# wamuumu/query-recommendation-system

Measured on AMD Instinct MI355X. Metric: MinHash signatures/sec through the whole hot path (signatures -> LSH candidates -> pair scoring -> top-K), higher is better.
Workload: dtype u16/int32 MinHash values, uint64 keys and pairs (integer); float64 cosine

## Files before the change

query-recommendation-system_amd/csrc/bucket.hip:

```cpp
#include "common.h"


struct PartPool {
  uint64_t *keys;
  uint32_t *vals;
  unsigned long long *cursor;
  uint32_t cap;
  uint4 *runs;
  unsigned long long *nruns;
  uint32_t runs_max;
  uint32_t *fill;
  uint32_t slot_base;
};

#ifndef QR_PS_IPT
#define QR_PS_IPT 16
#endif
constexpr int PS_IPT = QR_PS_IPT;
constexpr int PS_TILE = SORT_THREADS * PS_IPT;
constexpr int PS_WGS = PS_IPT <= 16 ? 3 : 2;
template <bool LEVEL2>
__global__ __launch_bounds__(SORT_THREADS, PS_WGS) void part_scatter_atomic_kernel(
    const uint64_t *__restrict__ keys_in, const uint32_t *__restrict__ vals_in, uint64_t *__restrict__ keys_out,
    uint32_t *__restrict__ vals_out, int64_t n_in, int ntiles, int shift, uint32_t dmask,
    uint32_t *__restrict__ cursors, uint32_t cap, uint32_t *__restrict__ overflow, uint64_t ek,
    const uint32_t *__restrict__ in_counts, uint32_t in_cap, int64_t chunk_len, int64_t chunk_stride,
    int64_t band_stride, PartPool pool) {
  __shared__ uint32_t cnt[RADIX];
  __shared__ uint32_t lsum[SORT_THREADS / WAVE];
  __shared__ uint32_t gdelta[RADIX];
  __shared__ uint8_t gok[RADIX];
  __shared__ uint64_t skey[PS_TILE];
  __shared__ uint32_t sval[PS_TILE];
  const int tile = LEVEL2 ? (int)blockIdx.x : xcd_tile(blockIdx.x, ntiles), batch = blockIdx.y;
  const int lane = threadIdx.x & (WAVE - 1), w = threadIdx.x >> 6;
  const int64_t n = LEVEL2 ? (int64_t)min(in_counts[batch], in_cap) : n_in;
  const int64_t tbase = (int64_t)tile * PS_TILE;
  if (tbase >= n) return;
  cnt[threadIdx.x] = 0;
  __syncthreads();
  const size_t boff = LEVEL2 ? (size_t)batch * in_cap : (size_t)batch * (size_t)(band_stride ? band_stride : n);
  const bool chunked = !LEVEL2 && chunk_len > 0 && chunk_len < n;
  const int64_t wbase = tbase + (int64_t)w * (WAVE * PS_IPT);
  const uint32_t nd = dmask + 1u;
  uint64_t key[PS_IPT];
  uint32_t val[PS_IPT];
  uint32_t dr[PS_IPT];
#pragma unroll
  for (int k = 0; k < PS_IPT; ++k) {
    const int64_t idx = wbase + (int64_t)k * WAVE + lane;
    const size_t at = chunked ? boff + (size_t)(idx / chunk_len) * chunk_stride + (size_t)(idx % chunk_len) : boff + idx;
    key[k] = idx < n ? keys_in[at] : ek;
    val[k] = LEVEL2 ? (idx < n ? vals_in[boff + idx] : 0u) : (uint32_t)idx;
  }
#pragma unroll
  for (int k = 0; k < PS_IPT; ++k) {
    const int64_t idx = wbase + (int64_t)k * WAVE + lane;
    const bool valid = idx < n && (LEVEL2 || key[k] != ek);
    if (!LEVEL2) key[k] = qr_mix64(key[k]);
    const uint32_t d = (uint32_t)(key[k] >> shift) & dmask;
    dr[k] = valid ? (d << 16) | atomicAdd(&cnt[d], 1u) : 0xFFFFFFFFu;
  }
  __syncthreads();
  const uint32_t tc = cnt[threadIdx.x];
  const uint32_t gb = tc ? atomicAdd(&cursors[(size_t)batch * nd + threadIdx.x], tc) : 0u;
  uint32_t lstart;
  {
    const uint32_t linc = wave_incl_scan(tc);
    if (lane == WAVE - 1) lsum[w] = linc;
    __syncthreads();
    lstart = linc - tc;
#pragma unroll
    for (int k = 0; k < SORT_THREADS / WAVE; ++k)
      if (k < w) lstart += lsum[k];
    cnt[threadIdx.x] = lstart;
  }
  __syncthreads();
#pragma unroll
  for (int k = 0; k < PS_IPT; ++k) {
    if (dr[k] != 0xFFFFFFFFu) {
      const uint32_t lp = cnt[dr[k] >> 16] + (dr[k] & 0xFFFFu);
      skey[lp] = key[k];
      sval[lp] = val[k];
    }
  }
  {
    const int d = threadIdx.x;
    uint32_t where = gb + tc <= cap ? 1u : 0u;
    uint32_t delta = (uint32_t)d * cap + gb - lstart;
    if (!where) {
      if (pool.keys) {
        const unsigned long long pb =
            __hip_atomic_fetch_add(pool.cursor, (unsigned long long)tc, __ATOMIC_RELAXED, __HIP_MEMORY_SCOPE_AGENT);
        if (pb + tc <= (unsigned long long)pool.cap) {
          const unsigned long long ri = __hip_atomic_fetch_add(pool.nruns, 1ull, __ATOMIC_RELAXED, __HIP_MEMORY_SCOPE_AGENT);
          if (ri < (unsigned long long)pool.runs_max) {
            const uint32_t slot = pool.slot_base + (uint32_t)batch * nd + (uint32_t)d;
            pool.runs[ri] = make_uint4(slot, tc, (uint32_t)pb, 0u);
            atomicMin(&pool.fill[slot], gb);
            where = 2u;
            delta = (uint32_t)pb - lstart;
          }
        }
      }
      if (!where) atomicOr(overflow, 1u);
    }
    gok[d] = (uint8_t)where;
    gdelta[d] = delta;
  }
  __syncthreads();
  uint32_t nstaged = 0;
#pragma unroll
  for (int k = 0; k < SORT_THREADS / WAVE; ++k) nstaged += lsum[k];
  const size_t obase = (size_t)batch * nd * cap;
#pragma unroll
  for (int k = 0; k < PS_IPT; ++k) {
    const uint32_t p = k * SORT_THREADS + threadIdx.x;
    if (p < nstaged) {
      const uint64_t x = skey[p];
      const uint32_t d = (uint32_t)(x >> shift) & dmask;
      const uint32_t where = gok[d];
      if (where == 1u) {
        const size_t dst = obase + (uint32_t)(gdelta[d] + p);
        keys_out[dst] = x;
        vals_out[dst] = sval[p];
      } else if (where == 2u) {
        const uint32_t dst = gdelta[d] + p;
        pool.keys[dst] = x;
        pool.vals[dst] = sval[p];
      }
    }
  }
}

#ifndef QR_FIN_THREADS
#define QR_FIN_THREADS 1024
#endif
#ifndef QR_FIN_CAP
#define QR_FIN_CAP 6144
#endif
constexpr int FIN_THREADS = QR_FIN_THREADS;
constexpr int FIN_CAP = QR_FIN_CAP;
constexpr int FIN_IPT = FIN_CAP / FIN_THREADS;
constexpr int FIN_SMALL_THREADS = 512, FIN_SMALL_CAP = 4096;
constexpr int FIN_SMALL_MEAN = 2800;

template <int CAP = FIN_CAP> __device__ static inline uint32_t fin_home(uint64_t key) {
  uint32_t h = (uint32_t)key * 0x9E3779B1u;
  h ^= h >> 15;
  h += (uint32_t)(key >> 32) * 0x85EBCA77u;
  h ^= h >> 13;
  h *= 0xC2B2AE3Du;
  return __umulhi(h, (uint32_t)CAP);
}

#ifndef QR_FIN_COOP
#define QR_FIN_COOP 16
#endif
constexpr uint32_t FIN_COOP = QR_FIN_COOP;
__device__ static inline void emit_run(uint64_t *__restrict__ dst, uint32_t pos, uint32_t me, const uint32_t *run,
                                       uint32_t run_off, uint32_t c) {
  if (c <= FIN_COOP) {
    for (uint32_t t = 0; t < c; ++t) {
      const uint32_t other = run[run_off + t];
      dst[pos + t] = (uint64_t)min(me, other) << 32 | max(me, other);
    }
  }
  uint64_t big = __ballot(c > FIN_COOP);
  const int lane = threadIdx.x & (WAVE - 1);
// ... 59 lines not shown

template <int IPT>
__device__ static inline void fin_layout(const uint32_t (&so)[IPT], const uint32_t (&ireg)[IPT], const uint32_t *start,
                                         uint32_t *grp) {
#pragma unroll
  for (int j = 0; j < IPT; ++j)
    if (so[j] != 0xFFFFFFFFu) grp[start[so[j] & 0xFFFFu] + (so[j] >> 16)] = ireg[j];
}

template <int IPT>
__device__ static inline void fin_emit(uint64_t *__restrict__ dst, uint32_t pos, const uint32_t (&so)[IPT],
                                       const uint32_t (&ireg)[IPT], const uint32_t *start, const uint32_t *grp) {
#pragma unroll
  for (int j = 0; j < IPT; ++j) {
    const bool rec = so[j] != 0xFFFFFFFFu;
    const uint32_t o = rec ? so[j] >> 16 : 0u;
    emit_run(dst, pos, ireg[j], grp, rec ? start[so[j] & 0xFFFFu] : 0u, o);
    pos += o;
  }
}

template <int THREADS = FIN_THREADS, int CAP = FIN_CAP>
__global__ __launch_bounds__(THREADS, THREADS >= 1024 ? 8 : 6) void bucket_finish_kernel(
    const uint64_t *__restrict__ keys, const uint32_t *__restrict__ ids, int nparts, uint64_t ek, uint64_t *__restrict__ blk,
    uint32_t *__restrict__ overflow, uint64_t *__restrict__ out, uint64_t capacity, const uint32_t *__restrict__ counts,
    uint32_t cap, uint64_t *__restrict__ biglist, unsigned long long *__restrict__ nbig, uint32_t big_max,
    uint32_t big_base) {
  constexpr int IPT = CAP / THREADS;
  static_assert(CAP % THREADS == 0 && CAP <= 65535, "image = whole records per thread, slots fit 16 bits");
  __shared__ unsigned long long gbase;
  __shared__ __attribute__((aligned(16))) unsigned long long tab[CAP];
  __shared__ uint32_t cnt[CAP];
  __shared__ uint32_t wsum[THREADS / WAVE];
  const int part = blockIdx.x, band = blockIdx.y;
  const int tid = threadIdx.x;
  const size_t bslot = (size_t)band * nparts + part;
  const uint32_t m = counts[bslot];
  const size_t first = bslot * cap;
  if (m > (uint32_t)CAP || m > cap) {
    if (tid == 0) fin_list_part(big_base + bslot, biglist, nbig, big_max, overflow);
    return;
  }
  if (m == 0) return;
  const uint64_t *k = keys + first;
  const uint32_t *id = ids + first;
  uint64_t kreg[IPT];
  uint32_t ireg[IPT];
#pragma unroll
  for (int j = 0; j < IPT; ++j) {
    const uint32_t i = tid + j * THREADS;
    kreg[j] = i < m ? k[i] : ek;
    ireg[j] = i < m ? id[i] : 0u;
  }
#pragma unroll
  for (int j = 0; j < IPT; ++j) {
    const uint32_t i = tid + j * THREADS;
    tab[i] = ek;
    cnt[i] = 0;
  }
  __syncthreads();
  uint32_t so[IPT];
  uint32_t mine = 0;
  uint32_t slot[IPT];
  unsigned long long seen[IPT];
#pragma unroll
  for (int j = 0; j < IPT; ++j) {
    slot[j] = fin_home<CAP>(kreg[j]);
    seen[j] = kreg[j] != ek
                  ? atomicCAS(&tab[slot[j]], (unsigned long long)ek, (unsigned long long)kreg[j])
                  : (unsigned long long)ek;
  }
#pragma unroll
  for (int j = 0; j < IPT; ++j) {
    if (kreg[j] != ek) {
      unsigned long long old = seen[j];
      while (old != ek && old != kreg[j]) {
        slot[j] = slot[j] + 1 == (uint32_t)CAP ? 0u : slot[j] + 1;
        old = atomicCAS(&tab[slot[j]], (unsigned long long)ek, (unsigned long long)kreg[j]);
      }
// ... 3 lines not shown
  for (int j = 0; j < IPT; ++j) {
    so[j] = 0xFFFFFFFFu;
    if (kreg[j] != ek) {
      const uint32_t o = atomicAdd(&cnt[slot[j]], 1u);
      so[j] = o << 16 | slot[j];
      mine += o;
    }
  }
  uint32_t tot;
  const uint32_t pos0 = fin_reserve<THREADS>(mine, wsum, blk, &gbase, tot);
  if (tot == 0) return;
  fin_run_starts<THREADS, IPT>([&](uint32_t sl) { return cnt[sl]; }, cnt, wsum);
  __syncthreads();
  uint32_t *grp = reinterpret_cast<uint32_t *>(tab);
  fin_layout(so, ireg, cnt, grp);
  __syncthreads();
  const uint64_t obase = (uint64_t)gbase;
  if (obase + tot > capacity) return;
  fin_emit(out + obase, pos0, so, ireg, cnt, grp);
}

constexpr int FIN_PK_THREADS = 512, FIN_PK_CAP = 4096, FIN_PK_MAX = 4095;
__global__ __launch_bounds__(FIN_PK_THREADS, 8) void bucket_finish_packed_kernel(
    const uint64_t *__restrict__ keys, const uint32_t *__restrict__ ids, int nparts, uint64_t *__restrict__ blk,
    uint32_t *__restrict__ overflow, uint64_t *__restrict__ out, uint64_t capacity, const uint32_t *__restrict__ counts,
    uint32_t cap, uint64_t *__restrict__ biglist, unsigned long long *__restrict__ nbig, uint32_t big_max,
    uint32_t big_base) {
  constexpr int THREADS = FIN_PK_THREADS, CAP = FIN_PK_CAP, IPT = CAP / THREADS;
  constexpr unsigned long long KMASK = (1ull << 52) - 1ull, ONE = 1ull << 52;
  __shared__ unsigned long long gbase;
  __shared__ __attribute__((aligned(16))) unsigned long long tab[CAP];
  __shared__ uint32_t wsum[THREADS / WAVE];
  const int part = blockIdx.x, band = blockIdx.y;
  const int tid = threadIdx.x;
  const size_t bslot = (size_t)band * nparts + part;
  const uint32_t m = counts[bslot];
  if (m > (uint32_t)FIN_PK_MAX) {
    if (tid == 0) fin_list_part(big_base + bslot, biglist, nbig, big_max, overflow);
    return;
  }
  if (m == 0) return;
  const size_t first = bslot * cap;
  const uint64_t *k = keys + first;
  const uint32_t *id = ids + first;
  uint64_t kreg[IPT];
  uint32_t ireg[IPT];
#pragma unroll
  for (int j = 0; j < IPT; ++j) {
    const uint32_t i = tid + j * THREADS;
    kreg[j] = i < m ? k[i] : 0ull;
    ireg[j] = i < m ? id[i] : 0u;
  }
#pragma unroll
  for (int j = 0; j < IPT; ++j) tab[tid + j * THREADS] = 0ull;
  __syncthreads();
  uint32_t so[IPT];
  uint32_t mine = 0;
#pragma unroll
  for (int j = 0; j < IPT; ++j) {
    so[j] = 0xFFFFFFFFu;
    if (tid + j * THREADS < (int)m) {
      const unsigned long long k52 = kreg[j] & KMASK;
      uint32_t slot = fin_home<CAP>(kreg[j]);
      uint32_t o;
      for (;;) {
        const unsigned long long old = atomicCAS(&tab[slot], 0ull, k52 | ONE);
        if (old == 0ull) {
          o = 0;
          break;
        }
        if ((old & KMASK) == k52) {
          o = (uint32_t)(atomicAdd(&tab[slot], ONE) >> 52);
          break;
        }
        slot = slot + 1 == (uint32_t)CAP ? 0u : slot + 1;
      }
      so[j] = o << 16 | slot;
      mine += o;
    }
  }
  uint32_t tot;
  const uint32_t pos0 = fin_reserve<THREADS>(mine, wsum, blk, &gbase, tot);
  if (tot == 0) return;
  uint32_t *rs = reinterpret_cast<uint32_t *>(tab);
  uint32_t *grp = rs + CAP;
  fin_run_starts<THREADS, IPT>([&](uint32_t sl) { return (uint32_t)(tab[sl] >> 52); }, rs, wsum);
  __syncthreads();
  fin_layout(so, ireg, rs, grp);
  __syncthreads();
  const uint64_t obase = (uint64_t)gbase;
  if (obase + tot > capacity) return;
  fin_emit(out + obase, pos0, so, ireg, rs, grp);
}

constexpr int FIN_BIG_GRID = 256;
constexpr int FIN_BIG_BLOCKS = 16;
constexpr uint32_t FIN_BIG_LIST = 4096;
constexpr int FIN_BIG_SLICES = 8;
constexpr int FIN_RANK_SORT = 256;
constexpr uint32_t POOL_RUNS = 1u << 20;

struct BigDesc {
  uint64_t where;
  uint32_t m, pool;
};

__global__ __launch_bounds__(256) void bucket_big_gather_kernel(const uint64_t *__restrict__ biglist,
                                                                const unsigned long long *__restrict__ nbig, uint32_t big_max,
                                                                BigDesc *__restrict__ desc, const uint64_t *__restrict__ part_keys,
                                                                const uint32_t *__restrict__ part_ids,
                                                                const uint32_t *__restrict__ counts, uint32_t cap, PartPool pool,
                                                                uint32_t max_records, uint32_t *__restrict__ overflow) {
  __shared__ unsigned long long base_s;
  __shared__ uint32_t match[256];
  __shared__ uint32_t nmatch;
  const int tid = threadIdx.x;
  unsigned long long nb = *nbig;
  if (nb > big_max) nb = big_max;
  for (unsigned long long e = blockIdx.x; e < nb; e += gridDim.x) {
    const uint32_t slot = (uint32_t)biglist[e];
    const uint32_t m = counts[slot];
    const uint32_t f = pool.fill ? pool.fill[slot] : 0xFFFFFFFFu;
    if (m > max_records || (f == 0xFFFFFFFFu && m > cap)) {
      if (tid == 0) {
        atomicOr(overflow, 1u);
        desc[e] = BigDesc{0ull, 0u, 0u};
      }
      continue;
    }
    if (f == 0xFFFFFFFFu) {
      if (tid == 0) desc[e] = BigDesc{(uint64_t)slot * cap, m, 0u};
      continue;
    }
// ... 22 lines not shown
      __syncthreads();
      const unsigned long long r = r0 + tid;
      if (r < nr && pool.runs[r].x == slot) match[atomicAdd(&nmatch, 1u)] = (uint32_t)r;
      __syncthreads();
      const uint32_t nm = nmatch;
      for (uint32_t q = 0; q < nm; ++q) {
        const uint4 run = pool.runs[match[q]];
        if (at + run.y <= m)
          for (uint32_t i = tid; i < run.y; i += blockDim.x) {
            pool.keys[base + at + i] = pool.keys[(size_t)run.z + i];
            pool.vals[base + at + i] = pool.vals[(size_t)run.z + i];
          }
        at += run.y;
      }
    }
    if (tid == 0) {
      if (at != m) atomicOr(overflow, 1u);
      desc[e] = BigDesc{(uint64_t)base, at == m ? m : 0u, 1u};
    }
  }
}

__global__ __launch_bounds__(FIN_THREADS) void bucket_finish_big_kernel(
    const uint64_t *__restrict__ keys, const uint32_t *__restrict__ ids, const uint64_t *pool_keys, const uint32_t *pool_ids,
    uint64_t ek, const BigDesc *__restrict__ desc, const unsigned long long *__restrict__ nbig, uint32_t big_max,
    uint64_t *__restrict__ blk, uint64_t *__restrict__ out, uint64_t capacity) {
  __shared__ unsigned long long gbase;
  __shared__ __attribute__((aligned(16))) unsigned long long tab[FIN_CAP];
  __shared__ uint32_t cnt[FIN_CAP + 1];
  __shared__ uint32_t grp[FIN_CAP];
  __shared__ uint32_t srt[FIN_CAP];
  __shared__ uint32_t wsum[FIN_THREADS / WAVE];
  __shared__ uint32_t lrun[FIN_CAP / (FIN_RANK_SORT + 1) + 1], nlrun;
  const int tid = threadIdx.x;
  unsigned long long nb = *nbig;
  if (nb > big_max) nb = big_max;
  constexpr int COMBOS = FIN_BIG_BLOCKS * (FIN_BIG_BLOCKS + 1) / 2;
  static_assert(FIN_THREADS % FIN_BIG_SLICES == 0, "a thread's records share their position mod the slice count");
  for (unsigned long long item = blockIdx.x; item < nb * COMBOS * FIN_BIG_SLICES; item += gridDim.x) {
    const uint32_t sl = (uint32_t)(item % FIN_BIG_SLICES);
    const unsigned long long e = item / ((unsigned long long)COMBOS * FIN_BIG_SLICES);
    int combo = (int)((item / FIN_BIG_SLICES) % COMBOS);
    uint32_t bi = 0;
    while (combo > (int)bi) {
      combo -= (int)bi + 1;
      ++bi;
    }
    const uint32_t bj_only = (uint32_t)combo;
    const BigDesc de = desc[e];
    const uint32_t m = de.m;
    const uint64_t *k = (de.pool ? pool_keys : keys) + de.where;
    const uint32_t *id = (de.pool ? pool_ids : ids) + de.where;
    const uint32_t nblk = (m + FIN_CAP - 1) / FIN_CAP;
    if (bi >= nblk) continue;
    {
      const uint32_t lo = bi * FIN_CAP, mb = min((uint32_t)FIN_CAP, m - lo);
      uint64_t kreg[FIN_IPT];
      uint32_t ireg[FIN_IPT], so[FIN_IPT];
      __syncthreads();
#pragma unroll
      for (int j = 0; j < FIN_IPT; ++j) {
        const uint32_t i = tid + j * FIN_THREADS;
        kreg[j] = i < mb ? k[lo + i] : ek;
        ireg[j] = i < mb ? id[lo + i] : 0u;
        tab[i] = ek;
        cnt[i] = 0;
      }
      __syncthreads();
#pragma unroll
      for (int j = 0; j < FIN_IPT; ++j) {
        so[j] = 0xFFFFFFFFu;
        if (kreg[j] != ek) {
          uint32_t slot = fin_home(kreg[j]);
          for (;;) {
            const unsigned long long old = atomicCAS(&tab[slot], (unsigned long long)ek, (unsigned long long)kreg[j]);
            if (old == ek || old == kreg[j]) break;
            slot = slot + 1 == (uint32_t)FIN_CAP ? 0u : slot + 1;
          }
          const uint32_t o = atomicAdd(&cnt[slot], 1u);
          so[j] = o << 16 | slot;
        }
      }
      __syncthreads();
      {
        const uint32_t all = fin_run_starts<FIN_THREADS, FIN_IPT>([&](uint32_t s) { return cnt[s]; }, cnt, wsum);
        if (tid == 0) cnt[FIN_CAP] = all;
      }
// ... 66 lines not shown
        const uint32_t pos0 = block_excl_scan<FIN_THREADS>(mine, wsum, tot);
        if (tid == 0 && tot)
          gbase = __hip_atomic_fetch_add(reinterpret_cast<unsigned long long *>(blk), (unsigned long long)tot,
                                         __ATOMIC_RELAXED, __HIP_MEMORY_SCOPE_AGENT);
        __syncthreads();
        if (tot && gbase + tot <= capacity) {
          uint64_t *dst = out + gbase;
          uint32_t pos = pos0;
#pragma unroll
          for (int j = 0; j < FIN_IPT; ++j) {
            emit_run(dst, pos, ireg[j], srt, so[j] != 0xFFFFFFFFu ? cnt[so[j] & 0xFFFFu] : 0u, rk[j]);
            pos += rk[j];
          }
        }
      }
      if (bj_only < bi) {
        const uint32_t bj = bj_only;
        const uint32_t lo2 = bj * FIN_CAP;
        uint32_t hit[FIN_IPT];
        uint32_t mine2 = 0;
#pragma unroll
        for (int j = 0; j < FIN_IPT; ++j) {
          const uint32_t i = tid + j * FIN_THREADS;
          const uint64_t x = k[lo2 + i];
          ireg[j] = id[lo2 + i];
          uint32_t slot = fin_home(x), found = 0xFFFFFFFFu;
          const bool my_slice = (uint32_t)(tid & (FIN_BIG_SLICES - 1)) == sl;
          for (int step = 0; my_slice && step < FIN_CAP; ++step) {
            const unsigned long long tv = tab[slot];
            if (tv == x) {
              found = slot;
              break;
            }
            if (tv == ek) break;
            slot = slot + 1 == (uint32_t)FIN_CAP ? 0u : slot + 1;
          }
          if ((uint32_t)(tid & (FIN_BIG_SLICES - 1)) != sl) found = 0xFFFFFFFFu;
          hit[j] = found;
          if (found != 0xFFFFFFFFu) mine2 += cnt[found + 1] - cnt[found];
        }
        uint32_t tot2;
        const uint32_t p0 = block_excl_scan<FIN_THREADS>(mine2, wsum, tot2);
        if (tid == 0 && tot2)
          gbase = __hip_atomic_fetch_add(reinterpret_cast<unsigned long long *>(blk), (unsigned long long)tot2,
                                         __ATOMIC_RELAXED, __HIP_MEMORY_SCOPE_AGENT);
        __syncthreads();
        if (tot2 && gbase + tot2 <= capacity) {
          uint64_t *dst = out + gbase;
          uint32_t pos = p0;
#pragma unroll
          for (int j = 0; j < FIN_IPT; ++j) {
            const bool h = hit[j] != 0xFFFFFFFFu;
            const uint32_t s0 = h ? cnt[hit[j]] : 0u, c = h ? cnt[hit[j] + 1] - s0 : 0u;
            emit_run(dst, pos, ireg[j], grp, s0, c);
            pos += c;
          }
        }
        __syncthreads();
      }
    }
  }
}

static uint32_t g_big_limit = (uint32_t)FIN_BIG_BLOCKS * FIN_CAP;
QRLSH_EXPORT int64_t qrlsh_set_big_part_limit(int64_t records) {
  const int64_t max = (int64_t)FIN_BIG_BLOCKS * FIN_CAP, old = g_big_limit;
  g_big_limit = (uint32_t)(records <= 0 || records > max ? max : records);
  return old;
}

static size_t align16(size_t x) { return (x + 15) & ~(size_t)15; }
static int coarse_bits(int T);
constexpr int EMIT_MAX_GROUPS = 2;
struct BucketWs {
  uint32_t *cur1, *counts;
  uint64_t *big;
  uint32_t *fill;
  unsigned long long *poolctl;
  uint4 *runs;
  BigDesc *desc;
  size_t bytes;
};
static BucketWs bucket_ws(void *workspace, int32_t b, int32_t T) {
  BucketWs w;
  const size_t slots = (size_t)b << T;
  char *p = static_cast<char *>(workspace);
  size_t off = 0;
  w.cur1 = reinterpret_cast<uint32_t *>(p + off);
  if (T > 8) off += align16(((size_t)b << coarse_bits(T)) * sizeof(uint32_t));
  w.counts = reinterpret_cast<uint32_t *>(p + off);
  off += align16(slots * sizeof(uint32_t));
  w.big = reinterpret_cast<uint64_t *>(p + off);
  off += slots * sizeof(uint64_t);
  w.fill = reinterpret_cast<uint32_t *>(p + off);
  off += align16(slots * sizeof(uint32_t));
  w.poolctl = reinterpret_cast<unsigned long long *>(p + off);
  off += 16;
  w.runs = reinterpret_cast<uint4 *>(p + off);
  off += (size_t)POOL_RUNS * sizeof(uint4);
  w.desc = reinterpret_cast<BigDesc *>(p + off);
  off += (size_t)EMIT_MAX_GROUPS * FIN_BIG_LIST * sizeof(BigDesc);
  w.bytes = off;
  return w;
}

QRLSH_EXPORT size_t qrlsh_bucket_workspace_bytes(int64_t nq, int32_t b, int32_t part_bits) {
  if (nq <= 0 || b <= 0 || part_bits < 8 || part_bits > 16) return 64;
  return bucket_ws(nullptr, b, part_bits).bytes;
}

static int bucket_check(const char *name, const uint64_t *keys, uint64_t *part_keys, uint32_t *part_ids,
                        uint64_t *tmp_keys, uint32_t *tmp_ids, int64_t nq, int32_t b, int32_t r, int32_t part_bits,
                        void *workspace, size_t workspace_bytes, uint64_t *total_overflow_out, hipStream_t st) {
  QR_CHECK_ARG(nq >= 0 && b > 0 && b <= 65535 && r > 0, "%s: bad sizes nq=%lld b=%d r=%d", name, (long long)nq, b, r);
  QR_CHECK_ARG(part_bits >= 8 && part_bits <= 16, "%s: part_bits=%d not in [8,16]", name, part_bits);
  QR_CHECK_ARG(nq < (1ll << 32), "%s: nq too large", name);
  QR_CHECK_ARG(total_overflow_out && workspace, "%s: null pointer", name);
  if (hipMemsetAsync(total_overflow_out, 0, 2 * sizeof(uint64_t), st) != hipSuccess) {
    qrlsh_set_error("%s: hipMemsetAsync failed", name);
    return QRLSH_EHIP;
  }
  if (nq == 0) return QRLSH_OK;
  QR_CHECK_ARG(keys && part_keys && part_ids, "%s: null pointer", name);
  QR_CHECK_ARG(part_bits == 8 || (tmp_keys && tmp_ids), "%s: part_bits > 8 needs tmp buffers", name);
  if (workspace_bytes < qrlsh_bucket_workspace_bytes(nq, b, part_bits)) {
    qrlsh_set_error("%s: workspace %zu < %zu bytes", name, workspace_bytes,
                    qrlsh_bucket_workspace_bytes(nq, b, part_bits));
    return QRLSH_EWORKSPACE;
  }
  return QRLSH_OK;
}
// ... 15 lines not shown
  const int64_t c = ((nq >> T) * 2 + 128 + 63) / 64 * 64;
  return (uint32_t)(c < FIN_CAP ? c : FIN_CAP);
}
static size_t pool_records(int64_t nq, int32_t b) {
  size_t n = (size_t)b * (size_t)nq / 16;
  if (n < ((size_t)1 << 20)) n = (size_t)1 << 20;
  if (n > 0xFFFFFF00ull) n = 0xFFFFFF00ull;
  return n;
}
static size_t region_words(int64_t nq, int32_t b, int32_t part_bits) {
  return part_bits == 8 ? (size_t)b * RADIX * part_region(nq) : ((size_t)b << part_bits) * fine_region(nq, part_bits);
}

QRLSH_EXPORT size_t qrlsh_bucket_part_words(int64_t nq, int32_t b, int32_t part_bits) {
  if (nq <= 0 || b <= 0) return 0;
  const size_t plain = (size_t)b * nq;
  const size_t regions = region_words(nq, b, part_bits) + pool_records(nq, b);
  return regions > plain ? regions : plain;
}
QRLSH_EXPORT size_t qrlsh_bucket_tmp_words(int64_t nq, int32_t b, int32_t part_bits) {
  if (nq <= 0 || b <= 0 || part_bits <= 8) return 0;
  const size_t plain = (size_t)b * nq;
  const int c1 = coarse_bits(part_bits);
  const size_t regions = ((size_t)b << c1) * coarse_region(nq, c1);
  return regions > plain ? regions : plain;
}

QRLSH_EXPORT int qrlsh_bucket_pairs_emit(const uint64_t *keys, uint64_t *part_keys, uint32_t *part_ids,
                                         uint64_t *tmp_keys, uint32_t *tmp_ids, int64_t nq, int32_t b, int32_t r,
                                         int32_t part_bits, void *workspace, size_t workspace_bytes,
                                         uint64_t *pairs_out, uint64_t capacity, uint64_t *total_overflow_out,
                                         void *stream) {
  return qrlsh_bucket_pairs_emit_chunked(keys, 0, 0, 0, part_keys, part_ids, tmp_keys, tmp_ids, nq, b, r, part_bits,
                                         workspace, workspace_bytes, pairs_out, capacity, total_overflow_out, stream);
}

QRLSH_EXPORT int qrlsh_bucket_pairs_emit_chunked(const uint64_t *keys, int64_t key_chunk, int64_t key_chunk_stride,
                                                 int64_t key_band_stride, uint64_t *part_keys, uint32_t *part_ids,
                                                 uint64_t *tmp_keys, uint32_t *tmp_ids, int64_t nq, int32_t b,
                                                 int32_t r, int32_t part_bits, void *workspace,
                                                 size_t workspace_bytes, uint64_t *pairs_out, uint64_t capacity,
                                                 uint64_t *total_overflow_out, void *stream) {
  QR_CHECK_ARG(key_chunk >= 0 && key_chunk_stride >= 0 && key_band_stride >= 0,
               "qrlsh_bucket_pairs_emit_chunked: bad key layout");
  hipStream_t st = static_cast<hipStream_t>(stream);
  const int rc = bucket_check("qrlsh_bucket_pairs_emit", keys, part_keys, part_ids, tmp_keys, tmp_ids, nq, b, r,
                              part_bits, workspace, workspace_bytes, total_overflow_out, st);
  if (rc != QRLSH_OK || nq == 0) return rc;
  QR_CHECK_ARG(pairs_out || capacity == 0, "qrlsh_bucket_pairs_emit: null output with capacity %llu",
               (unsigned long long)capacity);
  const int nparts = 1 << part_bits;
  const BucketWs w = bucket_ws(workspace, b, part_bits);
  const uint64_t ekx = qr_mix64(qr_empty_key(r));
#define QR_PART_SCATTER(LEVEL2_, ...) QR_LAUNCH("part_scatter", (part_scatter_atomic_kernel<LEVEL2_>), __VA_ARGS__)
  const int T = part_bits;
  const bool two = T > 8;
  const int c1 = two ? coarse_bits(T) : 8;
  const uint32_t cap1 = two ? coarse_region(nq, c1) : part_region(nq), cap2 = two ? fine_region(nq, T) : cap1;
  const uint32_t lowmask = (1u << (T - c1)) - 1u;
  uint32_t *cur1 = w.cur1, *cur2 = w.counts;
  if (hipMemsetAsync(cur1, 0, ((size_t)b << c1) * sizeof(uint32_t), st) != hipSuccess ||
      (two && hipMemsetAsync(cur2, 0, ((size_t)b << T) * sizeof(uint32_t), st) != hipSuccess)) {
    qrlsh_set_error("qrlsh_bucket_pairs_emit: hipMemsetAsync failed");
    return QRLSH_EHIP;
  }
  uint32_t *ovf = reinterpret_cast<uint32_t *>(total_overflow_out + 1);
  const size_t reg_words = region_words(nq, b, T);
  PartPool pool;
  pool.keys = part_keys + reg_words;
  pool.vals = part_ids + reg_words;
  pool.cursor = w.poolctl;
  pool.nruns = w.poolctl + 1;
  pool.cap = (uint32_t)pool_records(nq, b);
  pool.runs = w.runs;
  pool.runs_max = POOL_RUNS;
  pool.fill = w.fill;
  pool.slot_base = 0;
  PartPool no_pool = pool;
  no_pool.keys = nullptr;
  no_pool.vals = nullptr;
  if (hipMemsetAsync(w.fill, 0xFF, ((size_t)b << T) * sizeof(uint32_t), st) != hipSuccess ||
      hipMemsetAsync(w.poolctl, 0, 16, st) != hipSuccess) {
    qrlsh_set_error("qrlsh_bucket_pairs_emit: hipMemsetAsync failed");
    return QRLSH_EHIP;
  }
  constexpr int MAX_GROUPS = EMIT_MAX_GROUPS;
  unsigned long long *nbig0 = reinterpret_cast<unsigned long long *>(w.big);
  uint64_t *biglist0 = w.big + MAX_GROUPS;
  const uint64_t slots = (uint64_t)b << T;
  if (hipMemsetAsync(nbig0, 0, MAX_GROUPS * sizeof(unsigned long long), st) != hipSuccess) {
    qrlsh_set_error("qrlsh_bucket_pairs_emit: hipMemsetAsync failed");
    return QRLSH_EHIP;
  }
  const bool small_parts = two && small_form(nq, T);
  const int ntiles = (int)ceil_div64(nq, PS_TILE);
  const int64_t band_words = key_band_stride ? key_band_stride : nq;
  const int GROUPS = (int64_t)b * nq >= (64ll << 20) ? MAX_GROUPS : 1;
  const int per = (b + GROUPS - 1) / GROUPS;
  const int ngroups = (b + per - 1) / per;
  const uint64_t list_room = (slots - MAX_GROUPS) / (uint64_t)ngroups;
  const uint32_t big_max = (uint32_t)(list_room < FIN_BIG_LIST ? list_room : FIN_BIG_LIST);
  if (ngroups > 1 && hipMemsetAsync(w.runs, 0, (size_t)POOL_RUNS * sizeof(uint4), st) != hipSuccess) {
    qrlsh_set_error("qrlsh_bucket_pairs_emit: hipMemsetAsync failed");
    return QRLSH_EHIP;
  }
  hipStream_t aux = nullptr;
  int gi = 0;
  for (int g0 = 0; g0 < b; g0 += per, ++gi) {
    const int nb = (b - g0 < per) ? b - g0 : per;
    hipStream_t s = (aux && (gi & 1)) ? aux : st;
    uint64_t *biglist = biglist0 + (size_t)gi * big_max;
    unsigned long long *nbig = nbig0 + gi;
    uint64_t *k1 = two ? tmp_keys : part_keys;
    uint32_t *v1 = two ? tmp_ids : part_ids;
    pool.slot_base = (uint32_t)((size_t)g0 << T);
    BigDesc *desc = w.desc + (size_t)gi * FIN_BIG_LIST;
    QR_PART_SCATTER(false, dim3(ntiles, nb), dim3(SORT_THREADS), 0, s, keys + (size_t)g0 * band_words,
                    (const uint32_t *)nullptr, k1 + ((size_t)g0 << c1) * cap1, v1 + ((size_t)g0 << c1) * cap1, nq,
                    ntiles, 64 - c1, (1u << c1) - 1u, cur1 + ((size_t)g0 << c1), cap1, ovf, qr_empty_key(r),
                    (const uint32_t *)nullptr, 0u, key_chunk, key_chunk_stride, key_band_stride, two ? no_pool : pool);
    if (two)
      QR_PART_SCATTER(true, dim3((unsigned)ceil_div64(cap1, PS_TILE), nb << c1), dim3(SORT_THREADS), 0, s,
                      (const uint64_t *)tmp_keys + ((size_t)g0 << c1) * cap1,
                      (const uint32_t *)tmp_ids + ((size_t)g0 << c1) * cap1, part_keys + ((size_t)g0 << T) * cap2,
                      part_ids + ((size_t)g0 << T) * cap2, (int64_t)0, 0, 64 - T, lowmask, cur2 + ((size_t)g0 << T),
                      cap2, ovf, qr_empty_key(r), (const uint32_t *)cur1 + ((size_t)g0 << c1), cap1, (int64_t)0,
                      (int64_t)0, (int64_t)0, pool);
    if (gi == 0 && b > per) aux = qr_aux_fork(st);
    const uint32_t slot0 = (uint32_t)((size_t)g0 << T);
    const uint64_t *gkeys = part_keys + (size_t)slot0 * cap2;
    const uint32_t *gids = part_ids + (size_t)slot0 * cap2, *gcounts = cur2 + slot0;
    if (small_parts && T >= 12)
      QR_LAUNCH("bucket_emit", bucket_finish_packed_kernel, dim3(nparts, nb), dim3(FIN_PK_THREADS), 0, s, gkeys, gids, nparts,
                total_overflow_out, ovf, pairs_out, capacity, gcounts, cap2, biglist, nbig, big_max, slot0);
    else if (small_parts)
      QR_LAUNCH("bucket_emit", (bucket_finish_kernel<FIN_SMALL_THREADS, FIN_SMALL_CAP>), dim3(nparts, nb),
                dim3(FIN_SMALL_THREADS), 0, s, gkeys, gids, nparts, ekx, total_overflow_out, ovf, pairs_out, capacity, gcounts,
                cap2, biglist, nbig, big_max, slot0);
    else
      QR_LAUNCH("bucket_emit", (bucket_finish_kernel<>), dim3(nparts, nb), dim3(FIN_THREADS), 0, s, gkeys, gids, nparts, ekx,
                total_overflow_out, ovf, pairs_out, capacity, gcounts, cap2, biglist, nbig, big_max, slot0);
    QR_LAUNCH("bucket_emit_big", bucket_big_gather_kernel, dim3(64), dim3(256), 0, s, (const uint64_t *)biglist,
              (const unsigned long long *)nbig, big_max, desc, (const uint64_t *)part_keys, (const uint32_t *)part_ids,
              (const uint32_t *)cur2, cap2, pool, g_big_limit, ovf);
    QR_LAUNCH("bucket_emit_big", bucket_finish_big_kernel, dim3(FIN_BIG_GRID), dim3(FIN_THREADS), 0, s,
              (const uint64_t *)part_keys, (const uint32_t *)part_ids, (const uint64_t *)pool.keys,
              (const uint32_t *)pool.vals, ekx, (const BigDesc *)desc, (const unsigned long long *)nbig, big_max,
              total_overflow_out, pairs_out, capacity);
  }
  if (aux && qr_aux_join(st) != QRLSH_OK) return QRLSH_EHIP;
  QR_LAUNCH_CHECK("qrlsh_bucket_pairs_emit");
  return QRLSH_OK;
#undef QR_PART_SCATTER
}
```

Before: 608.8 million.

## Pack record ids into key high bits and store 16-bit id tails

```diff
diff --git a/query-recommendation-system_amd/csrc/bucket.hip b/query-recommendation-system_amd/csrc/bucket.hip
--- a/query-recommendation-system_amd/csrc/bucket.hip
+++ b/query-recommendation-system_amd/csrc/bucket.hip
@@ -1,9 +1,17 @@
 #include "common.h"
 
+
+__device__ static inline uint64_t rec_x(uint64_t word, int xbits) { return word & ((1ull << xbits) - 1ull); }
+__device__ static inline uint64_t rec_word(uint64_t x, uint32_t id_hi, int xbits) {
+  return rec_x(x, xbits) | (uint64_t)id_hi << xbits;
+}
+__device__ static inline uint32_t rec_id(uint64_t word, uint16_t tail, int xbits) {
+  return (uint32_t)(word >> xbits) << 16 | tail;
+}
 
 struct PartPool {
   uint64_t *keys;
-  uint32_t *vals;
+  uint16_t *vals;
   unsigned long long *cursor;
   uint32_t cap;
   uint4 *runs;
@@ -18,20 +26,21 @@
 #endif
 constexpr int PS_IPT = QR_PS_IPT;
 constexpr int PS_TILE = SORT_THREADS * PS_IPT;
+static_assert(65536 % PS_TILE == 0, "a tile of the first step lies in one slab and its records share id >> 16");
 constexpr int PS_WGS = PS_IPT <= 16 ? 3 : 2;
 template <bool LEVEL2>
 __global__ __launch_bounds__(SORT_THREADS, PS_WGS) void part_scatter_atomic_kernel(
-    const uint64_t *__restrict__ keys_in, const uint32_t *__restrict__ vals_in, uint64_t *__restrict__ keys_out,
-    uint32_t *__restrict__ vals_out, int64_t n_in, int ntiles, int shift, uint32_t dmask,
+    const uint64_t *__restrict__ keys_in, const uint16_t *__restrict__ tails_in, uint64_t *__restrict__ keys_out,
+    uint16_t *__restrict__ tails_out, int64_t n_in, int ntiles, int shift, uint32_t dmask,
     uint32_t *__restrict__ cursors, uint32_t cap, uint32_t *__restrict__ overflow, uint64_t ek,
     const uint32_t *__restrict__ in_counts, uint32_t in_cap, int64_t chunk_len, int64_t chunk_stride,
-    int64_t band_stride, PartPool pool) {
+    int64_t band_stride, int c1, int nslabs, int slab_shift, PartPool pool) {
   __shared__ uint32_t cnt[RADIX];
   __shared__ uint32_t lsum[SORT_THREADS / WAVE];
   __shared__ uint32_t gdelta[RADIX];
   __shared__ uint8_t gok[RADIX];
   __shared__ uint64_t skey[PS_TILE];
-  __shared__ uint32_t sval[PS_TILE];
+  __shared__ uint16_t sval[PS_TILE];
   const int tile = LEVEL2 ? (int)blockIdx.x : xcd_tile(blockIdx.x, ntiles), batch = blockIdx.y;
   const int lane = threadIdx.x & (WAVE - 1), w = threadIdx.x >> 6;
   const int64_t n = LEVEL2 ? (int64_t)min(in_counts[batch], in_cap) : n_in;
@@ -39,19 +48,28 @@
   if (tbase >= n) return;
   cnt[threadIdx.x] = 0;
   __syncthreads();
+  uint32_t obatch, id_hi;
+  if (LEVEL2) {
+    const uint32_t bs = (uint32_t)batch >> c1, band = bs / (uint32_t)nslabs, slab = bs - band * (uint32_t)nslabs;
+    obatch = band << c1 | ((uint32_t)batch & ((1u << c1) - 1u));
+    id_hi = slab << c1;
+  } else {
+    obatch = (uint32_t)batch * (uint32_t)nslabs + (uint32_t)(tbase >> slab_shift);
+    id_hi = (uint32_t)(tbase >> 16) & dmask;
+  }
   const size_t boff = LEVEL2 ? (size_t)batch * in_cap : (size_t)batch * (size_t)(band_stride ? band_stride : n);
   const bool chunked = !LEVEL2 && chunk_len > 0 && chunk_len < n;
   const int64_t wbase = tbase + (int64_t)w * (WAVE * PS_IPT);
   const uint32_t nd = dmask + 1u;
   uint64_t key[PS_IPT];
-  uint32_t val[PS_IPT];
+  uint16_t val[PS_IPT];
   uint32_t dr[PS_IPT];
 #pragma unroll
   for (int k = 0; k < PS_IPT; ++k) {
     const int64_t idx = wbase + (int64_t)k * WAVE + lane;
     const size_t at = chunked ? boff + (size_t)(idx / chunk_len) * chunk_stride + (size_t)(idx % chunk_len) : boff + idx;
     key[k] = idx < n ? keys_in[at] : ek;
-    val[k] = LEVEL2 ? (idx < n ? vals_in[boff + idx] : 0u) : (uint32_t)idx;
+    val[k] = LEVEL2 ? (idx < n ? tails_in[boff + idx] : (uint16_t)0) : (uint16_t)idx;
   }
 #pragma unroll
   for (int k = 0; k < PS_IPT; ++k) {
@@ -63,7 +81,7 @@
   }
   __syncthreads();
   const uint32_t tc = cnt[threadIdx.x];
-  const uint32_t gb = tc ? atomicAdd(&cursors[(size_t)batch * nd + threadIdx.x], tc) : 0u;
+  const uint32_t gb = tc ? atomicAdd(&cursors[(size_t)obatch * nd + threadIdx.x], tc) : 0u;
   uint32_t lstart;
   {
     const uint32_t linc = wave_incl_scan(tc);
@@ -95,7 +113,7 @@
         if (pb + tc <= (unsigned long long)pool.cap) {
           const unsigned long long ri = __hip_atomic_fetch_add(pool.nruns, 1ull, __ATOMIC_RELAXED, __HIP_MEMORY_SCOPE_AGENT);
           if (ri < (unsigned long long)pool.runs_max) {
-            const uint32_t slot = pool.slot_base + (uint32_t)batch * nd + (uint32_t)d;
+            const uint32_t slot = pool.slot_base + obatch * nd + (uint32_t)d;
             pool.runs[ri] = make_uint4(slot, tc, (uint32_t)pb, 0u);
             atomicMin(&pool.fill[slot], gb);
             where = 2u;
@@ -112,7 +130,7 @@
   uint32_t nstaged = 0;
 #pragma unroll
   for (int k = 0; k < SORT_THREADS / WAVE; ++k) nstaged += lsum[k];
-  const size_t obase = (size_t)batch * nd * cap;
+  const size_t obase = (size_t)obatch * nd * cap;
 #pragma unroll
   for (int k = 0; k < PS_IPT; ++k) {
     const uint32_t p = k * SORT_THREADS + threadIdx.x;
@@ -120,13 +138,14 @@
       const uint64_t x = skey[p];
       const uint32_t d = (uint32_t)(x >> shift) & dmask;
       const uint32_t where = gok[d];
+      const uint64_t word = rec_word(x, LEVEL2 ? id_hi | (uint32_t)(x >> (64 - c1)) : id_hi, shift);
       if (where == 1u) {
         const size_t dst = obase + (uint32_t)(gdelta[d] + p);
-        keys_out[dst] = x;
-        vals_out[dst] = sval[p];
+        keys_out[dst] = word;
+        tails_out[dst] = sval[p];
       } else if (where == 2u) {
         const uint32_t dst = gdelta[d] + p;
-        pool.keys[dst] = x;
+        pool.keys[dst] = word;
         pool.vals[dst] = sval[p];
       }
     }
@@ -145,6 +164,7 @@
 constexpr int FIN_SMALL_THREADS = 512, FIN_SMALL_CAP = 4096;
 constexpr int FIN_SMALL_MEAN = 2800;
 
+constexpr unsigned long long FIN_FREE = ~0ull;
 template <int CAP = FIN_CAP> __device__ static inline uint32_t fin_home(uint64_t key) {
   uint32_t h = (uint32_t)key * 0x9E3779B1u;
   h ^= h >> 15;
@@ -250,11 +270,12 @@
 
 template <int THREADS = FIN_THREADS, int CAP = FIN_CAP>
 __global__ __launch_bounds__(THREADS, THREADS >= 1024 ? 8 : 6) void bucket_finish_kernel(
-    const uint64_t *__restrict__ keys, const uint32_t *__restrict__ ids, int nparts, uint64_t ek, uint64_t *__restrict__ blk,
+    const uint64_t *__restrict__ keys, const uint16_t *__restrict__ tails, int nparts, int xbits, uint64_t *__restrict__ blk,
     uint32_t *__restrict__ overflow, uint64_t *__restrict__ out, uint64_t capacity, const uint32_t *__restrict__ counts,
     uint32_t cap, uint64_t *__restrict__ biglist, unsigned long long *__restrict__ nbig, uint32_t big_max,
     uint32_t big_base) {
   constexpr int IPT = CAP / THREADS;
+  constexpr uint64_t ek = FIN_FREE;
   static_assert(CAP % THREADS == 0 && CAP <= 65535, "image = whole records per thread, slots fit 16 bits");
   __shared__ unsigned long long gbase;
   __shared__ __attribute__((aligned(16))) unsigned long long tab[CAP];
@@ -271,18 +292,22 @@
   }
   if (m == 0) return;
   const uint64_t *k = keys + first;
-  const uint32_t *id = ids + first;
+  const uint16_t *tl = tails + first;
   uint64_t kreg[IPT];
   uint32_t ireg[IPT];
 #pragma unroll
   for (int j = 0; j < IPT; ++j) {
     const uint32_t i = tid + j * THREADS;
     kreg[j] = i < m ? k[i] : ek;
-    ireg[j] = i < m ? id[i] : 0u;
+    ireg[j] = i < m ? tl[i] : 0u;
   }
 #pragma unroll
   for (int j = 0; j < IPT; ++j) {
     const uint32_t i = tid + j * THREADS;
+    if (i < m) {
+      ireg[j] = rec_id(kreg[j], (uint16_t)ireg[j], xbits);
+      kreg[j] = rec_x(kreg[j], xbits);
+    }
     tab[i] = ek;
     cnt[i] = 0;
   }
@@ -332,7 +357,7 @@
 
 constexpr int FIN_PK_THREADS = 512, FIN_PK_CAP = 4096, FIN_PK_MAX = 4095;
 __global__ __launch_bounds__(FIN_PK_THREADS, 8) void bucket_finish_packed_kernel(
-    const uint64_t *__restrict__ keys, const uint32_t *__restrict__ ids, int nparts, uint64_t *__restrict__ blk,
+    const uint64_t *__restrict__ keys, const uint16_t *__restrict__ tails, int nparts, int xbits, uint64_t *__restrict__ blk,
     uint32_t *__restrict__ overflow, uint64_t *__restrict__ out, uint64_t capacity, const uint32_t *__restrict__ counts,
     uint32_t cap, uint64_t *__restrict__ biglist, unsigned long long *__restrict__ nbig, uint32_t big_max,
     uint32_t big_base) {
@@ -352,14 +377,14 @@
   if (m == 0) return;
   const size_t first = bslot * cap;
   const uint64_t *k = keys + first;
-  const uint32_t *id = ids + first;
+  const uint16_t *tl = tails + first;
   uint64_t kreg[IPT];
   uint32_t ireg[IPT];
 #pragma unroll
   for (int j = 0; j < IPT; ++j) {
     const uint32_t i = tid + j * THREADS;
     kreg[j] = i < m ? k[i] : 0ull;
-    ireg[j] = i < m ? id[i] : 0u;
+    ireg[j] = i < m ? tl[i] : 0u;
   }
 #pragma unroll
   for (int j = 0; j < IPT; ++j) tab[tid + j * THREADS] = 0ull;
@@ -370,8 +395,9 @@
   for (int j = 0; j < IPT; ++j) {
     so[j] = 0xFFFFFFFFu;
     if (tid + j * THREADS < (int)m) {
-      const unsigned long long k52 = kreg[j] & KMASK;
-      uint32_t slot = fin_home<CAP>(kreg[j]);
+      const unsigned long long k52 = rec_x(kreg[j], xbits);
+      ireg[j] = rec_id(kreg[j], (uint16_t)ireg[j], xbits);
+      uint32_t slot = fin_home<CAP>(k52);
       uint32_t o;
       for (;;) {
         const unsigned long long old = atomicCAS(&tab[slot], 0ull, k52 | ONE);
@@ -418,7 +444,7 @@
 __global__ __launch_bounds__(256) void bucket_big_gather_kernel(const uint64_t *__restrict__ biglist,
                                                                 const unsigned long long *__restrict__ nbig, uint32_t big_max,
                                                                 BigDesc *__restrict__ desc, const uint64_t *__restrict__ part_keys,
-                                                                const uint32_t *__restrict__ part_ids,
+                                                                const uint16_t *__restrict__ part_ids,
                                                                 const uint32_t *__restrict__ counts, uint32_t cap, PartPool pool,
                                                                 uint32_t max_records, uint32_t *__restrict__ overflow) {
   __shared__ unsigned long long base_s;
@@ -487,8 +513,8 @@
 }
 
 __global__ __launch_bounds__(FIN_THREADS) void bucket_finish_big_kernel(
-    const uint64_t *__restrict__ keys, const uint32_t *__restrict__ ids, const uint64_t *pool_keys, const uint32_t *pool_ids,
-    uint64_t ek, const BigDesc *__restrict__ desc, const unsigned long long *__restrict__ nbig, uint32_t big_max,
+    const uint64_t *__restrict__ keys, const uint16_t *__restrict__ ids, const uint64_t *pool_keys, const uint16_t *pool_ids,
+    int xbits, const BigDesc *__restrict__ desc, const unsigned long long *__restrict__ nbig, uint32_t big_max,
     uint64_t *__restrict__ blk, uint64_t *__restrict__ out, uint64_t capacity) {
   __shared__ unsigned long long gbase;
   __shared__ __attribute__((aligned(16))) unsigned long long tab[FIN_CAP];
@@ -498,6 +524,7 @@
   __shared__ uint32_t wsum[FIN_THREADS / WAVE];
   __shared__ uint32_t lrun[FIN_CAP / (FIN_RANK_SORT + 1) + 1], nlrun;
   const int tid = threadIdx.x;
+  constexpr uint64_t ek = FIN_FREE;
   unsigned long long nb = *nbig;
   if (nb > big_max) nb = big_max;
   constexpr int COMBOS = FIN_BIG_BLOCKS * (FIN_BIG_BLOCKS + 1) / 2;
@@ -515,7 +542,7 @@
     const BigDesc de = desc[e];
     const uint32_t m = de.m;
     const uint64_t *k = (de.pool ? pool_keys : keys) + de.where;
-    const uint32_t *id = (de.pool ? pool_ids : ids) + de.where;
+    const uint16_t *id = (de.pool ? pool_ids : ids) + de.where;
     const uint32_t nblk = (m + FIN_CAP - 1) / FIN_CAP;
     if (bi >= nblk) continue;
     {
@@ -526,8 +553,13 @@
 #pragma unroll
       for (int j = 0; j < FIN_IPT; ++j) {
         const uint32_t i = tid + j * FIN_THREADS;
-        kreg[j] = i < mb ? k[lo + i] : ek;
-        ireg[j] = i < mb ? id[lo + i] : 0u;
+        kreg[j] = ek;
+        ireg[j] = 0u;
+        if (i < mb) {
+          const uint64_t word = k[lo + i];
+          kreg[j] = rec_x(word, xbits);
+          ireg[j] = rec_id(word, id[lo + i], xbits);
+        }
         tab[i] = ek;
         cnt[i] = 0;
       }
@@ -640,8 +672,8 @@
 #pragma unroll
         for (int j = 0; j < FIN_IPT; ++j) {
           const uint32_t i = tid + j * FIN_THREADS;
-          const uint64_t x = k[lo2 + i];
-          ireg[j] = id[lo2 + i];
+          const uint64_t word = k[lo2 + i], x = rec_x(word, xbits);
+          ireg[j] = rec_id(word, id[lo2 + i], xbits);
           uint32_t slot = fin_home(x), found = 0xFFFFFFFFu;
           const bool my_slice = (uint32_t)(tid & (FIN_BIG_SLICES - 1)) == sl;
           for (int step = 0; my_slice && step < FIN_CAP; ++step) {
@@ -687,35 +719,40 @@
   return old;
 }
 
+static int coarse_bits(int T);
+static int slab_bits(int T) { return 16 + coarse_bits(T); }
+static int n_slabs(int64_t nq, int T) { return T > 8 ? (int)((nq + (1ll << slab_bits(T)) - 1) >> slab_bits(T)) : 1; }
+
 static size_t align16(size_t x) { return (x + 15) & ~(size_t)15; }
-static int coarse_bits(int T);
 constexpr int EMIT_MAX_GROUPS = 2;
 struct BucketWs {
+  uint32_t *fill;
   uint32_t *cur1, *counts;
-  uint64_t *big;
-  uint32_t *fill;
-  unsigned long long *poolctl;
+  unsigned long long *nbig, *poolctl;
   uint4 *runs;
+  uint64_t *biglist;
   BigDesc *desc;
   size_t bytes;
 };
-static BucketWs bucket_ws(void *workspace, int32_t b, int32_t T) {
+static BucketWs bucket_ws(void *workspace, int64_t nq, int32_t b, int32_t T) {
   BucketWs w;
   const size_t slots = (size_t)b << T;
   char *p = static_cast<char *>(workspace);
   size_t off = 0;
+  w.fill = reinterpret_cast<uint32_t *>(p + off);
+  off += align16(slots * sizeof(uint32_t));
   w.cur1 = reinterpret_cast<uint32_t *>(p + off);
-  if (T > 8) off += align16(((size_t)b << coarse_bits(T)) * sizeof(uint32_t));
+  if (T > 8) off += align16((((size_t)b * n_slabs(nq, T)) << coarse_bits(T)) * sizeof(uint32_t));
   w.counts = reinterpret_cast<uint32_t *>(p + off);
   off += align16(slots * sizeof(uint32_t));
-  w.big = reinterpret_cast<uint64_t *>(p + off);
-  off += slots * sizeof(uint64_t);
-  w.fill = reinterpret_cast<uint32_t *>(p + off);
-  off += align16(slots * sizeof(uint32_t));
+  w.nbig = reinterpret_cast<unsigned long long *>(p + off);
+  off += align16(EMIT_MAX_GROUPS * sizeof(unsigned long long));
   w.poolctl = reinterpret_cast<unsigned long long *>(p + off);
   off += 16;
   w.runs = reinterpret_cast<uint4 *>(p + off);
   off += (size_t)POOL_RUNS * sizeof(uint4);
+  w.biglist = reinterpret_cast<uint64_t *>(p + off);
+  off += align16(slots * sizeof(uint64_t));
   w.desc = reinterpret_cast<BigDesc *>(p + off);
   off += (size_t)EMIT_MAX_GROUPS * FIN_BIG_LIST * sizeof(BigDesc);
   w.bytes = off;
@@ -724,7 +761,7 @@
 
 QRLSH_EXPORT size_t qrlsh_bucket_workspace_bytes(int64_t nq, int32_t b, int32_t part_bits) {
   if (nq <= 0 || b <= 0 || part_bits < 8 || part_bits > 16) return 64;
-  return bucket_ws(nullptr, b, part_bits).bytes;
+  return bucket_ws(nullptr, nq, b, part_bits).bytes;
 }
 
 static int bucket_check(const char *name, const uint64_t *keys, uint64_t *part_keys, uint32_t *part_ids,
@@ -786,7 +823,8 @@
   if (nq <= 0 || b <= 0 || part_bits <= 8) return 0;
   const size_t plain = (size_t)b * nq;
   const int c1 = coarse_bits(part_bits);
-  const size_t regions = ((size_t)b << c1) * coarse_region(nq, c1);
+  const int64_t slab = 1ll << slab_bits(part_bits);
+  const size_t regions = (((size_t)b * n_slabs(nq, part_bits)) << c1) * coarse_region(nq < slab ? nq : slab, c1);
   return regions > plain ? regions : plain;
 }
 
@@ -813,26 +851,30 @@
   if (rc != QRLSH_OK || nq == 0) return rc;
   QR_CHECK_ARG(pairs_out || capacity == 0, "qrlsh_bucket_pairs_emit: null output with capacity %llu",
                (unsigned long long)capacity);
+  uint32_t *ovf = reinterpret_cast<uint32_t *>(total_overflow_out + 1);
+  if (nq > (1ll << (16 + part_bits))) {
+    if (hipMemsetAsync(ovf, 1, 1, st) != hipSuccess) {
+      qrlsh_set_error("qrlsh_bucket_pairs_emit: hipMemsetAsync failed");
+      return QRLSH_EHIP;
+    }
+    return QRLSH_OK;
+  }
   const int nparts = 1 << part_bits;
-  const BucketWs w = bucket_ws(workspace, b, part_bits);
-  const uint64_t ekx = qr_mix64(qr_empty_key(r));
+  const BucketWs w = bucket_ws(workspace, nq, b, part_bits);
 #define QR_PART_SCATTER(LEVEL2_, ...) QR_LAUNCH("part_scatter", (part_scatter_atomic_kernel<LEVEL2_>), __VA_ARGS__)
   const int T = part_bits;
   const bool two = T > 8;
   const int c1 = two ? coarse_bits(T) : 8;
-  const uint32_t cap1 = two ? coarse_region(nq, c1) : part_region(nq), cap2 = two ? fine_region(nq, T) : cap1;
+  const int nslabs = n_slabs(nq, T), slab_shift = two ? slab_bits(T) : 63;
+  const int64_t slab_nq = two && nq > (1ll << slab_shift) ? 1ll << slab_shift : nq;
+  const uint32_t cap1 = two ? coarse_region(slab_nq, c1) : part_region(nq), cap2 = two ? fine_region(nq, T) : cap1;
   const uint32_t lowmask = (1u << (T - c1)) - 1u;
   uint32_t *cur1 = w.cur1, *cur2 = w.counts;
-  if (hipMemsetAsync(cur1, 0, ((size_t)b << c1) * sizeof(uint32_t), st) != hipSuccess ||
-      (two && hipMemsetAsync(cur2, 0, ((size_t)b << T) * sizeof(uint32_t), st) != hipSuccess)) {
-    qrlsh_set_error("qrlsh_bucket_pairs_emit: hipMemsetAsync failed");
-    return QRLSH_EHIP;
-  }
-  uint32_t *ovf = reinterpret_cast<uint32_t *>(total_overflow_out + 1);
+  uint16_t *part_tails = reinterpret_cast<uint16_t *>(part_ids), *tmp_tails = reinterpret_cast<uint16_t *>(tmp_ids);
   const size_t reg_words = region_words(nq, b, T);
   PartPool pool;
   pool.keys = part_keys + reg_words;
-  pool.vals = part_ids + reg_words;
+  pool.vals = part_tails + reg_words;
   pool.cursor = w.poolctl;
   pool.nruns = w.poolctl + 1;
   pool.cap = (uint32_t)pool_records(nq, b);
@@ -843,19 +885,10 @@
   PartPool no_pool = pool;
   no_pool.keys = nullptr;
   no_pool.vals = nullptr;
-  if (hipMemsetAsync(w.fill, 0xFF, ((size_t)b << T) * sizeof(uint32_t), st) != hipSuccess ||
-      hipMemsetAsync(w.poolctl, 0, 16, st) != hipSuccess) {
-    qrlsh_set_error("qrlsh_bucket_pairs_emit: hipMemsetAsync failed");
-    return QRLSH_EHIP;
-  }
   constexpr int MAX_GROUPS = EMIT_MAX_GROUPS;
-  unsigned long long *nbig0 = reinterpret_cast<unsigned long long *>(w.big);
-  uint64_t *biglist0 = w.big + MAX_GROUPS;
+  unsigned long long *nbig0 = w.nbig;
+  uint64_t *biglist0 = w.biglist;
   const uint64_t slots = (uint64_t)b << T;
-  if (hipMemsetAsync(nbig0, 0, MAX_GROUPS * sizeof(unsigned long long), st) != hipSuccess) {
-    qrlsh_set_error("qrlsh_bucket_pairs_emit: hipMemsetAsync failed");
-    return QRLSH_EHIP;
-  }
   const bool small_parts = two && small_form(nq, T);
   const int ntiles = (int)ceil_div64(nq, PS_TILE);
   const int64_t band_words = key_band_stride ? key_band_stride : nq;
@@ -864,7 +897,12 @@
   const int ngroups = (b + per - 1) / per;
   const uint64_t list_room = (slots - MAX_GROUPS) / (uint64_t)ngroups;
   const uint32_t big_max = (uint32_t)(list_room < FIN_BIG_LIST ? list_room : FIN_BIG_LIST);
-  if (ngroups > 1 && hipMemsetAsync(w.runs, 0, (size_t)POOL_RUNS * sizeof(uint4), st) != hipSuccess) {
+  if (hipMemsetAsync(cur1, 0, (((size_t)b * nslabs) << c1) * sizeof(uint32_t), st) != hipSuccess ||
+      (two && hipMemsetAsync(cur2, 0, ((size_t)b << T) * sizeof(uint32_t), st) != hipSuccess) ||
+      hipMemsetAsync(w.fill, 0xFF, ((size_t)b << T) * sizeof(uint32_t), st) != hipSuccess ||
+      hipMemsetAsync(w.poolctl, 0, 16, st) != hipSuccess ||
+      hipMemsetAsync(nbig0, 0, MAX_GROUPS * sizeof(unsigned long long), st) != hipSuccess ||
+      (ngroups > 1 && hipMemsetAsync(w.runs, 0, (size_t)POOL_RUNS * sizeof(uint4), st) != hipSuccess)) {
     qrlsh_set_error("qrlsh_bucket_pairs_emit: hipMemsetAsync failed");
     return QRLSH_EHIP;
   }
@@ -876,40 +914,41 @@
     uint64_t *biglist = biglist0 + (size_t)gi * big_max;
     unsigned long long *nbig = nbig0 + gi;
     uint64_t *k1 = two ? tmp_keys : part_keys;
-    uint32_t *v1 = two ? tmp_ids : part_ids;
+    uint16_t *v1 = two ? tmp_tails : part_tails;
     pool.slot_base = (uint32_t)((size_t)g0 << T);
     BigDesc *desc = w.desc + (size_t)gi * FIN_BIG_LIST;
+    const size_t in0 = ((size_t)g0 * nslabs) << c1;
     QR_PART_SCATTER(false, dim3(ntiles, nb), dim3(SORT_THREADS), 0, s, keys + (size_t)g0 * band_words,
-                    (const uint32_t *)nullptr, k1 + ((size_t)g0 << c1) * cap1, v1 + ((size_t)g0 << c1) * cap1, nq,
-                    ntiles, 64 - c1, (1u << c1) - 1u, cur1 + ((size_t)g0 << c1), cap1, ovf, qr_empty_key(r),
-                    (const uint32_t *)nullptr, 0u, key_chunk, key_chunk_stride, key_band_stride, two ? no_pool : pool);
+                    (const uint16_t *)nullptr, k1 + in0 * cap1, v1 + in0 * cap1, nq, ntiles, 64 - c1, (1u << c1) - 1u,
+                    cur1 + in0, cap1, ovf, qr_empty_key(r), (const uint32_t *)nullptr, 0u, key_chunk, key_chunk_stride,
+                    key_band_stride, c1, nslabs, slab_shift, two ? no_pool : pool);
     if (two)
-      QR_PART_SCATTER(true, dim3((unsigned)ceil_div64(cap1, PS_TILE), nb << c1), dim3(SORT_THREADS), 0, s,
-                      (const uint64_t *)tmp_keys + ((size_t)g0 << c1) * cap1,
-                      (const uint32_t *)tmp_ids + ((size_t)g0 << c1) * cap1, part_keys + ((size_t)g0 << T) * cap2,
-                      part_ids + ((size_t)g0 << T) * cap2, (int64_t)0, 0, 64 - T, lowmask, cur2 + ((size_t)g0 << T),
-                      cap2, ovf, qr_empty_key(r), (const uint32_t *)cur1 + ((size_t)g0 << c1), cap1, (int64_t)0,
-                      (int64_t)0, (int64_t)0, pool);
+      QR_PART_SCATTER(true, dim3((unsigned)ceil_div64(cap1, PS_TILE), (nb * nslabs) << c1), dim3(SORT_THREADS), 0, s,
+                      (const uint64_t *)tmp_keys + in0 * cap1, (const uint16_t *)tmp_tails + in0 * cap1,
+                      part_keys + ((size_t)g0 << T) * cap2, part_tails + ((size_t)g0 << T) * cap2, (int64_t)0, 0, 64 - T,
+                      lowmask, cur2 + ((size_t)g0 << T), cap2, ovf, qr_empty_key(r), (const uint32_t *)cur1 + in0, cap1,
+                      (int64_t)0, (int64_t)0, (int64_t)0, c1, nslabs, slab_shift, pool);
     if (gi == 0 && b > per) aux = qr_aux_fork(st);
     const uint32_t slot0 = (uint32_t)((size_t)g0 << T);
     const uint64_t *gkeys = part_keys + (size_t)slot0 * cap2;
-    const uint32_t *gids = part_ids + (size_t)slot0 * cap2, *gcounts = cur2 + slot0;
+    const uint16_t *gids = part_tails + (size_t)slot0 * cap2;
+    const uint32_t *gcounts = cur2 + slot0;
     if (small_parts && T >= 12)
       QR_LAUNCH("bucket_emit", bucket_finish_packed_kernel, dim3(nparts, nb), dim3(FIN_PK_THREADS), 0, s, gkeys, gids, nparts,
-                total_overflow_out, ovf, pairs_out, capacity, gcounts, cap2, biglist, nbig, big_max, slot0);
+                64 - T, total_overflow_out, ovf, pairs_out, capacity, gcounts, cap2, biglist, nbig, big_max, slot0);
     else if (small_parts)
       QR_LAUNCH("bucket_emit", (bucket_finish_kernel<FIN_SMALL_THREADS, FIN_SMALL_CAP>), dim3(nparts, nb),
-                dim3(FIN_SMALL_THREADS), 0, s, gkeys, gids, nparts, ekx, total_overflow_out, ovf, pairs_out, capacity, gcounts,
+                dim3(FIN_SMALL_THREADS), 0, s, gkeys, gids, nparts, 64 - T, total_overflow_out, ovf, pairs_out, capacity, gcounts,
                 cap2, biglist, nbig, big_max, slot0);
     else
-      QR_LAUNCH("bucket_emit", (bucket_finish_kernel<>), dim3(nparts, nb), dim3(FIN_THREADS), 0, s, gkeys, gids, nparts, ekx,
+      QR_LAUNCH("bucket_emit", (bucket_finish_kernel<>), dim3(nparts, nb), dim3(FIN_THREADS), 0, s, gkeys, gids, nparts, 64 - T,
                 total_overflow_out, ovf, pairs_out, capacity, gcounts, cap2, biglist, nbig, big_max, slot0);
     QR_LAUNCH("bucket_emit_big", bucket_big_gather_kernel, dim3(64), dim3(256), 0, s, (const uint64_t *)biglist,
-              (const unsigned long long *)nbig, big_max, desc, (const uint64_t *)part_keys, (const uint32_t *)part_ids,
+              (const unsigned long long *)nbig, big_max, desc, (const uint64_t *)part_keys, (const uint16_t *)part_tails,
               (const uint32_t *)cur2, cap2, pool, g_big_limit, ovf);
     QR_LAUNCH("bucket_emit_big", bucket_finish_big_kernel, dim3(FIN_BIG_GRID), dim3(FIN_THREADS), 0, s,
-              (const uint64_t *)part_keys, (const uint32_t *)part_ids, (const uint64_t *)pool.keys,
-              (const uint32_t *)pool.vals, ekx, (const BigDesc *)desc, (const unsigned long long *)nbig, big_max,
+              (const uint64_t *)part_keys, (const uint16_t *)part_tails, (const uint64_t *)pool.keys,
+              (const uint16_t *)pool.vals, 64 - T, (const BigDesc *)desc, (const unsigned long long *)nbig, big_max,
               total_overflow_out, pairs_out, capacity);
   }
   if (aux && qr_aux_join(st) != QRLSH_OK) return QRLSH_EHIP;
```

New measurement: 626.3 million (median of 6 runs). +2.9%, better.
